# IBM/AdaMML

Measured on AMD Instinct MI355X. Metric: clips/sec (train fwd+bwd) RGB+Audio AdaMML @224^2, 5 seg, higher is better.
Workload: dtype bf16

## Files before the change

adamml_amd/csrc/conv_gemm.hip:

```cpp
#include "common.h"
#include "../../include/adamml_hip.h"
#include <type_traits>
#include <stdlib.h>
#include <stdio.h>


namespace {

constexpr int BP = 128;
constexpr int BK = 32;
constexpr int NTHREADS = 256;

struct ConvP {
    const bf16_t* x;
    const bf16_t* w;
    const float* in_scale;
    const float* in_shift;
    bf16_t* y;
    double* stats;
    int N, H, W, Cin, OH, OW, Cout, KH, KW, stride, pad, up, up_shift, act, accumulate;
    int P, K, cin_shift, n_ptiles, n_ctiles, tpb;
    size_t gx, gy;
    int in_gstride;
    const bf16_t* bn_z;
    const float* bn_vec;
    int bn_act;
    const bf16_t* res_out;
    const uint8_t* res_mask;
    int res_act;
    const bf16_t* bn_z2;
    const float* bn_vec2;
    double* stats2;
    const bf16_t* x2;
    const float* aff;
    bf16_t* side;
    const bf16_t* xb;
    int K1, C2;
    size_t gw;
    const float* epi_add;
    const float* id_scale;
    const float* id_shift;
    int id_gstride;
    uint8_t* mask_out;
    const bf16_t* pf_a;
    const float* pf_scale;
    const float* pf_shift;
    float* pf_ws;
    int pf_act, pf_gs, pf_nsplit;
    int wK;
    int cls_nt;
    unsigned cls_code;
    int oH, oW, o_ph, o_pw;
    int tp_nblk, tp_Q;
    bf16_t* tp_y;
    uint16_t* tp_code;
};

__device__ __forceinline__ int lds_off(int row, int chunk) {
    return row * 64 + ((chunk ^ (((row >> 3) & 1) << 1)) << 4);
}

template <int N, class F>
__device__ __forceinline__ void static_for(F&& f) {
    if constexpr (N > 0) {
        static_for<N - 1>(f);
        f(std::integral_constant<int, N - 1>{});
    }
}

template <int CH>
__device__ __forceinline__ int tr_swz(int row) {
    if (CH >= 128) return ((row & 3) | (((row >> 3) & 1) << 2)) << 2;
    return (((row >> 1) & 1) | (((row >> 3) & 1) << 1)) << 2;
}

__device__ const uint4 g_zero_page[4] = {};

__device__ __forceinline__ void glds16(const void* gsrc, unsigned lds_dst_uniform) {
    unsigned keep;
    asm volatile("s_mov_b32 %0, m0\n\ts_mov_b32 m0, %2\n\ts_nop 0\n\tglobal_load_lds_dwordx4 %1, off\n\ts_mov_b32 m0, %0"
                 : "=&s"(keep) : "v"(gsrc), "s"(lds_dst_uniform) : "memory");
}

constexpr int conv_gemm_wg_per_cu(int BC, int MODE, int PD, bool RES, bool DUAL, bool CAT, bool FADD, bool GLDS, int EID, int EPI) {
    if (RES || DUAL || CAT || EID) return 2;
    const int n = PD == 1 ? (BC == 128 ? 3 : 4) : (BC == 128 ? 2 : 3);
    const bool fewer = (MODE == 2 && !(BC == 128 && PD == 3)) || FADD ||
                       (BC == 64 && PD == 1 && ((EPI == 1 && !(MODE == 0 && GLDS)) || (EPI == 2 && MODE == 1))) ||
                       (BC == 128 && MODE == 1 && EPI == 2 && !GLDS);
    return fewer ? n - 1 : n;
}

template <int BC, int MODE, int PD, bool RES = false, bool DUAL = false, bool CAT = false, bool FADD = false, bool GLDS = false, int EID = 0,
          bool LZF = false, int EPI = -1, bool PF = false, int TP = 0>
__global__ __launch_bounds__(NTHREADS, conv_gemm_wg_per_cu(BC, MODE, PD, RES, DUAL, CAT, FADD, GLDS, EID, EPI)) void conv_gemm_kernel(ConvP p) {
    static_assert(TP == 0 || (FADD && EID && MODE == 0 && BC == 128 && (TP == 2 || TP == 4 || TP == 8)), "TP: FADD + EID, 128-wide cout tiles");
    constexpr int PPF = TP ? BP / TP : BP;
    constexpr int WCT = BC / 32;
    constexpr int WROWS = BC / 64;
    constexpr int TILE_BYTES = (BP + BC) * 64;
    constexpr int EPI_BYTES = BP * (BC * 2 + 16);
    constexpr int NBUF = GLDS ? 3 : 2;
    constexpr int STAGE_BYTES = (NBUF * TILE_BYTES) > EPI_BYTES ? (NBUF * TILE_BYTES) : EPI_BYTES;
    constexpr int NSR = (FADD || EPI == 0) ? 1 : 4;
    constexpr int CS_BYTES = NSR * 2 * BC * 4;
    constexpr int CS2_OFF = STAGE_BYTES + CS_BYTES + (MODE == 0 ? 0 : 256) + (MODE == 3 ? BP * 4 + 16 : 0);
    constexpr int VEC_MAXK = 1024;
    constexpr int VEC_OFF = CS2_OFF + (RES ? CS_BYTES : 0);
    constexpr int LZF_MAXK = 512;
    constexpr int PF_C = 64;
    constexpr int PF_OFF = (VEC_OFF + (LZF ? 2 * LZF_MAXK * 4 : (MODE == 0 && !GLDS) ? (DUAL ? 3 : 2) * VEC_MAXK * 4 : 0) + 1023) / 1024 * 1024;
    constexpr int SMEM_BYTES = PF ? PF_OFF + BP * PF_C * 2 : VEC_OFF + (LZF ? 2 * LZF_MAXK * 4 : (MODE == 0 && !GLDS) ? (DUAL ? 3 : 2) * VEC_MAXK * 4 : 0);
    __shared__ __attribute__((aligned(1024))) char smem[SMEM_BYTES];

    {
        const int g = blockIdx.y;
        p.x += (size_t)g * p.gx;
        p.y += (size_t)g * p.gy;
        if (p.stats) p.stats += (size_t)g * ADAMML_STAT_SLOTS * 2 * p.Cout;
        if (p.in_scale) { p.in_scale += (size_t)g * p.in_gstride; p.in_shift += (size_t)g * p.in_gstride; }
        if (p.bn_z) { p.bn_z += (size_t)g * p.gy; p.bn_vec += (size_t)g * 4 * p.Cout; }
        if (CAT) {
            p.xb += (size_t)g * (p.gx / p.K1) * p.C2;
            p.w += (size_t)g * p.gw;
            p.epi_add += (size_t)g * p.Cout;
        }
        if (DUAL) {
            p.x2 += (size_t)g * p.gx;
            p.aff += (size_t)g * 3 * p.K;
            if (p.side) p.side += (size_t)g * p.gx;
        }
        if (FADD) {
            p.bn_vec += (size_t)g * 4 * p.Cout;
            if (p.res_out) p.res_out += (size_t)g * p.gy;
            if (p.mask_out) p.mask_out += ((size_t)g * p.gy) >> 3;
            if (p.id_scale) { p.id_scale += (size_t)g * p.id_gstride; p.id_shift += (size_t)g * p.id_gstride; }
            if (TP) { p.tp_y += (size_t)g * (p.gy >> 1); if (p.tp_code) p.tp_code += ((size_t)g * (p.gy >> 1)) >> 3; }
        }
        if (PF) {
            p.pf_a += (size_t)g * p.P * PF_C;
            if (p.pf_scale) { p.pf_scale += (size_t)g * p.pf_gs; p.pf_shift += (size_t)g * p.pf_gs; }
        }
        if (RES) {
            p.res_out += (size_t)g * p.gy;
            if (p.res_mask) p.res_mask += ((size_t)g * p.gy) >> 3;
            if (p.bn_z2) { p.bn_z2 += (size_t)g * p.gy; p.bn_vec2 += (size_t)g * 4 * p.Cout; p.stats2 += (size_t)g * ADAMML_STAT_SLOTS * 2 * p.Cout; }
        }
    }
    const int tid = threadIdx.x;
    float* s_vec = reinterpret_cast<float*>(smem + (MODE == 0 ? VEC_OFF : 0));
    const int nvec = CAT ? p.C2 : p.K;
    const bool vec_lds = MODE == 0 && nvec <= VEC_MAXK && (DUAL || p.in_scale != nullptr);
    if (LZF) {
        const int kpad = (p.K + BK - 1) / BK * BK;
        for (int i = tid; i < kpad; i += NTHREADS) {
            s_vec[i] = i < p.K ? p.in_scale[i] : 0.f;
            s_vec[LZF_MAXK + i] = i < p.K ? p.in_shift[i] : 0.f;
        }
        __syncthreads();
    } else
    if (vec_lds) {
        if (DUAL) {
            for (int i = tid; i < 3 * p.K; i += NTHREADS) s_vec[i] = p.aff[i];
        } else {
            for (int i = tid; i < nvec; i += NTHREADS) { s_vec[i] = p.in_scale[i]; s_vec[nvec + i] = p.in_shift[i]; }
        }
        __syncthreads();
    }
    const int lane = tid & 63;
    const int wave = tid >> 6;
    const int wp = wave & 1;
    const int wc = wave >> 1;

    const int nwg = gridDim.x;
    int bid = blockIdx.x;
    {
        const int q = nwg >> 3, r = nwg & 7, xcd = bid & 7, idx = bid >> 3;
        bid = (xcd < r ? xcd * (q + 1) : r * (q + 1) + (xcd - r) * q) + idx;
    }
    const int ctile = bid % p.n_ctiles;
    const int pgrp = bid / p.n_ctiles;
    const int c0 = ctile * BC;

    const int chunk = tid & 3;
    const int row_a = tid >> 2;
    int* s_tapoff = reinterpret_cast<int*>(smem + STAGE_BYTES + CS_BYTES);
    int* s_wtap = s_tapoff + 64;
    int* s_orow = s_wtap + 4;
    if (MODE == 1) {
        if (tid < p.KH * p.KW) {
            const int kh = tid / p.KW, kw = tid - kh * p.KW;
            s_tapoff[tid] = (kh * p.W + kw) * p.Cin;
        }
    }
    if (MODE == 3) {
        if (tid < p.cls_nt) {
            const unsigned code = (p.cls_code >> (8 * tid)) & 0xffu;
            s_tapoff[tid] = ((int)(code & 1) * p.W + (int)((code >> 1) & 1)) * p.Cin;
            s_wtap[tid] = (int)(code >> 2) * p.Cin;
        }
    }
    const bf16_t* wrow[WROWS];
    bool w_ok[WROWS];
#pragma unroll
    for (int r = 0; r < WROWS; ++r) {
        int co = c0 + row_a + r * 64;
        w_ok[r] = co < p.Cout;
        wrow[r] = p.w + (size_t)(w_ok[r] ? co : 0) * p.wK;
    }
    const int li = lane & 15, lg = lane >> 4;
    constexpr int CROW = BC * 2 + 16;
    static_assert(BP * CROW <= STAGE_BYTES, "epilogue tile must fit the staging buffers");
    float* cs = reinterpret_cast<float*>(smem + STAGE_BYTES);
    float* cs2 = reinterpret_cast<float*>(smem + CS2_OFF);
    const bool second = RES && p.bn_z2 != nullptr;
    const bool epi_bnz = EPI < 0 ? p.bn_z != nullptr : EPI == 1;
    const bool epi_acc = EPI < 0 ? p.accumulate != 0 : (EPI == 2 && p.accumulate != 0);
    if (p.stats) {
        for (int i = tid; i < NSR * 2 * BC; i += NTHREADS) cs[i] = 0.f;
        if (second)
            for (int i = tid; i < NSR * 2 * BC; i += NTHREADS) cs2[i] = 0.f;
    }
    constexpr int CPR = BC / 8;
    constexpr int RSTEP = NTHREADS / CPR;
    const int ech = tid % CPR, erow0 = tid / CPR;
    const int eco = c0 + ech * 8;

    f32x4 pacc[PF ? 4 : 1][PF ? 2 : 1];
// ... 492 lines not shown
                if constexpr (EID != 0) {
                    dr[j] = eid[b0 + j];
                    mbits[j] = embits[b0 + j];
                } else {
                if (p.bn_z) zr[j] = __builtin_nontemporal_load(reinterpret_cast<const bf16x8*>(p.bn_z + pr[j]));
                if (p.accumulate) dr[j] = __builtin_nontemporal_load(reinterpret_cast<const bf16x8*>(p.y + pr[j]));
                if (p.res_mask) mbits[j] = p.res_mask[pr[j] >> 3];
                else orr[j] = __builtin_nontemporal_load(reinterpret_cast<const bf16x8*>(p.res_out + pr[j]));
                if (second) z2r[j] = __builtin_nontemporal_load(reinterpret_cast<const bf16x8*>(p.bn_z2 + pr[j]));
                }
            }
#pragma unroll
            for (int j = 0; j < EB; ++j) {
                const int r = erow0 + (b0 + j) * RSTEP;
                f32x8 f = bf8_to_f32(*reinterpret_cast<const bf16x8*>(smem + r * CROW + ech * 16));
                if (EID || p.accumulate) f += bf8_to_f32(dr[j]);
                if (EID || p.res_mask) {
#pragma unroll
                    for (int i = 0; i < 8; ++i) f[i] = (mbits[j] >> i) & 1u ? f[i] : 0.f;
                } else {
                    const f32x8 ov = bf8_to_f32(orr[EID ? 0 : j]);
#pragma unroll
                    for (int i = 0; i < 8; ++i) f[i] *= mask_act(ov[i], rlo, rhi);
                }
                const bf16x8 v = f32_to_bf8(f);
                if (ok[j]) *reinterpret_cast<bf16x8*>(p.y + pr[j]) = v;
                if constexpr (PF)
                    *reinterpret_cast<bf16x8*>(smem + r * CROW + ech * 16) = ok[j] ? v : bf16x8{0, 0, 0, 0, 0, 0, 0, 0};
                const float keep = ok[j] ? 1.f : 0.f;
                f = bf8_to_f32(v) * keep;
                esum += f;
                if constexpr (EID == 0) {
                if (p.bn_z) {
                    const f32x8 zv = bf8_to_f32(zr[j]);
#pragma unroll
                    for (int i = 0; i < 8; ++i) esq[i] += f[i] * (zv[i] - mu[i]) * is[i];
                }
                if (second) {
                    const f32x8 z2 = bf8_to_f32(z2r[j]);
#pragma unroll
                    for (int i = 0; i < 8; ++i) esq2[i] += f[i] * (z2[i] - mu2[i]) * is2[i];
                }
                }
            }
        }
        }
    } else if (eco < p.Cout && epi_bnz) {
        const f32x8 sc = load_f32x8(p.bn_vec + eco), sh = load_f32x8(p.bn_vec + p.Cout + eco);
        const f32x8 mu = load_f32x8(p.bn_vec + 2 * p.Cout + eco), is = load_f32x8(p.bn_vec + 3 * p.Cout + eco);
        f32x8 cadd;
#pragma unroll
        for (int i = 0; i < 8; ++i) cadd[i] = 0.f;
        if (CAT) cadd = load_f32x8(p.epi_add + eco);
        constexpr int NRZ = BP / RSTEP, EBZ = (EPI == 1 || CAT || DUAL) ? (NRZ < 4 ? NRZ : 4) : 1;
#pragma unroll 1
        for (int b0 = 0; b0 < NRZ; b0 += EBZ) {
            bf16x8 zrow[EBZ];
#pragma unroll
            for (int j = 0; j < EBZ; ++j) {
                const int r = erow0 + (b0 + j) * RSTEP;
                const int rc = p0 + r < p.P ? r : 0;
                const size_t pp = MODE == 3 ? (size_t)s_orow[rc] : (size_t)(p0 + rc);
                zrow[j] = *reinterpret_cast<const bf16x8*>(p.bn_z + pp * p.Cout + eco);
            }
#pragma unroll
            for (int j = 0; j < EBZ; ++j) {
                const int r = erow0 + (b0 + j) * RSTEP;
                if (p0 + r < p.P) {
                    const size_t pp = MODE == 3 ? (size_t)s_orow[r] : (size_t)(p0 + r);
                    f32x8 f = bf8_to_f32(*reinterpret_cast<const bf16x8*>(smem + r * CROW + ech * 16)) + cadd;
                    const f32x8 zv = bf8_to_f32(zrow[j]);
#pragma unroll
                    for (int i = 0; i < 8; ++i) f[i] *= act_mask(fmaf(zv[i], sc[i], sh[i]), p.bn_act);
                    const bf16x8 v = f32_to_bf8(f);
                    *reinterpret_cast<bf16x8*>(p.y + pp * p.Cout + eco) = v;
                    f = bf8_to_f32(v);
                    esum += f;
#pragma unroll
                    for (int i = 0; i < 8; ++i) esq[i] += f[i] * (zv[i] - mu[i]) * is[i];
                }
            }
        }
    } else if (eco < p.Cout) {
        constexpr int NRA = BP / RSTEP, EBA = (EPI == 2 || CAT || DUAL) ? (NRA < 4 ? NRA : 4) : 1;
#pragma unroll 1
        for (int b0 = 0; b0 < NRA; b0 += EBA) {
            bf16x8 arow[EBA];
            if (epi_acc) {
#pragma unroll
                for (int j = 0; j < EBA; ++j) {
                    const int r = erow0 + (b0 + j) * RSTEP;
                    const int rc = p0 + r < p.P ? r : 0;
                    const size_t pp = MODE == 3 ? (size_t)s_orow[rc] : (size_t)(p0 + rc);
                    arow[j] = *reinterpret_cast<const bf16x8*>(p.y + pp * p.Cout + eco);
                }
            }
#pragma unroll
            for (int j = 0; j < EBA; ++j) {
                const int r = erow0 + (b0 + j) * RSTEP;
                if (p0 + r < p.P) {
                    const size_t pp = MODE == 3 ? (size_t)s_orow[r] : (size_t)(p0 + r);
                    bf16x8 v = *reinterpret_cast<const bf16x8*>(smem + r * CROW + ech * 16);
                    f32x8 f = bf8_to_f32(v);
                    if (CAT) {
                        f += load_f32x8(p.epi_add + eco);
                        v = f32_to_bf8(f);
                    }
// ... 67 lines not shown
            }
        };
        static_assert(NSR == 4 || EPI == 0 || FADD, "VALU-folded sums need one row per wave");
        fold(esum, esq, cs);
        if (second) fold(esum, esq2, cs2);
    }
    if constexpr (PF) {
        __syncthreads();
        const int trow = 8 * lg + (li >> 2), tq = li & 3;
        const int x_lo = tr_swz<64>(trow), x_hi = tr_swz<64>(trow + 4);
        const float plo = p.pf_scale ? act_lo(p.pf_act) : -INFINITY, phi = p.pf_scale ? act_hi(p.pf_act) : INFINITY;
#pragma unroll
        for (int ks = 0; ks < BP / 32; ++ks) {
            bf16x8 fa[4], fb[2];
#pragma unroll
            for (int t = 0; t < 4; ++t) {
                const char* fp = smem + (ks * 32 + trow) * CROW + (wp * 64 + t * 16 + 4 * tq) * 2;
                union { s16x4 h[2]; bf16x8 v; } f;
                f.h[0] = __builtin_amdgcn_ds_read_tr16_b64_v4i16((__attribute__((address_space(3))) s16x4*)(fp));
                f.h[1] = __builtin_amdgcn_ds_read_tr16_b64_v4i16((__attribute__((address_space(3))) s16x4*)(fp + 4 * CROW));
                fa[t] = f.v;
            }
#pragma unroll
            for (int t = 0; t < 2; ++t) {
                const char* base = smem + PF_OFF + ks * 32 * 128;
                const int u = (wc * 32 + t * 16) / 4 + tq;
                union { s16x4 h[2]; bf16x8 v; } f;
                f.h[0] = __builtin_amdgcn_ds_read_tr16_b64_v4i16((__attribute__((address_space(3))) s16x4*)(base + trow * 128 + ((u ^ x_lo) << 3)));
                f.h[1] = __builtin_amdgcn_ds_read_tr16_b64_v4i16((__attribute__((address_space(3))) s16x4*)(base + (trow + 4) * 128 + ((u ^ x_hi) << 3)));
                f32x8 q = bf8_to_f32(f.v);
#pragma unroll
                for (int i = 0; i < 8; ++i) q[i] = clamp_act(fmaf(q[i], pfs[t], pfh[t]), plo, phi);
                fb[t] = f32_to_bf8(q);
            }
#pragma unroll
            for (int mt = 0; mt < 4; ++mt)
#pragma unroll
                for (int nt = 0; nt < 2; ++nt) pacc[mt][nt] = __builtin_amdgcn_mfma_f32_16x16x32_bf16(fa[mt], fb[nt], pacc[mt][nt], 0, 0, 0);
        }
    }
    __syncthreads();
    }
    if constexpr (PF) {
        float* out = p.pf_ws + (((size_t)blockIdx.y * p.n_ctiles + ctile) * p.pf_nsplit + pgrp) * (BC * PF_C);
#pragma unroll
        for (int mt = 0; mt < 4; ++mt)
#pragma unroll
            for (int nt = 0; nt < 2; ++nt)
#pragma unroll
                for (int r = 0; r < 4; ++r) out[(size_t)(wp * 64 + mt * 16 + lg * 4 + r) * PF_C + wc * 32 + nt * 16 + li] = pacc[mt][nt][r];
    }
    if (p.stats) {
        __syncthreads();
        const unsigned slot = blockIdx.x & (ADAMML_STAT_SLOTS - 1);
        for (int i = tid; i < 2 * BC; i += NTHREADS) {
            const int c = i < BC ? i : i - BC;
            if (c0 + c < p.Cout) {
                const size_t e = (i < BC ? 0 : (size_t)p.Cout) + c0 + c;
                float v = cs[i];
#pragma unroll
                for (int w = 1; w < NSR; ++w) v += cs[w * 2 * BC + i];
                stat_publish(p.stats + e, 2 * (size_t)p.Cout, slot, v);
                if (second) {
                    float v2 = cs2[i];
#pragma unroll
                    for (int w = 1; w < NSR; ++w) v2 += cs2[w * 2 * BC + i];
                    stat_publish(p.stats2 + e, 2 * (size_t)p.Cout, slot, v2);
                }
            }
        }
    }
}

struct WgradP {
    const bf16_t* dz;
    const bf16_t* x;
    const float* in_scale;
    const float* in_shift;
    float* dw;
    float* ws;
    size_t dw_numel;
    int nsplit;
    int N, H, W, Cin, OH, OW, Cout, KH, KW, stride, pad, act, cin_true;
    int P, pix_per_block, n_cotiles, n_tiles, cin_shift, NK;
    size_t gdz, gx;
    int in_gstride;
    const float* dz_scale;
    const float* dz_shift;
    int dz_act, dz_gstride;
};


template <int BM, int BN, int WPD = 1, bool LZ = false>
__global__ __launch_bounds__(NTHREADS) void conv_wgrad_kernel(WgradP p) {
    constexpr int AROW = BM * 2;
    constexpr int BROW = BN * 2;
    constexpr int TILE_BYTES = 32 * (AROW + BROW);
    constexpr int MT = BM / 32, NT = BN / 32;
    __shared__ __attribute__((aligned(16))) char smem[2 * TILE_BYTES];

    const int lb = (int)xcd_contiguous(blockIdx.x, gridDim.x);
    const int tile = lb % p.n_tiles;
    const int unit = lb / p.n_tiles;
    const int split = unit % p.nsplit, grp = unit / p.nsplit;
    p.dz += (size_t)grp * p.gdz;
    p.x += (size_t)grp * p.gx;
    if (p.in_scale) { p.in_scale += (size_t)grp * p.in_gstride; p.in_shift += (size_t)grp * p.in_gstride; }
// ... 553 lines not shown
    }
}

void launch_wgrad_reduce(const float* ws, float* dw, size_t n, int nsplit, int taps, int cin, int store, int groups, hipStream_t stream) {
    static const bool wide = !(getenv("ADAMML_REDUCE4") && getenv("ADAMML_REDUCE4")[0] == '0');
    if (wide && n % 4 == 0 && (reinterpret_cast<uintptr_t>(ws) & 15) == 0)
        hipLaunchKernelGGL(wgrad_reduce4_kernel, dim3((unsigned)((n / 4 + 15) / 16), groups), dim3(256), 0, stream, ws, dw, n, nsplit, taps, cin, store);
    else
        hipLaunchKernelGGL(wgrad_reduce_kernel, dim3((unsigned)((n + 15) / 16), groups), dim3(256), 0, stream, ws, dw, n, nsplit, taps, cin, store);
}

int ilog2_exact(int v) {
    int s = 0;
    while ((1 << s) < v) ++s;
    return (1 << s) == v ? s : -1;
}

}

bool adamml_conv3x3_c64_supported(const adamml_conv_desc_t* d);
bool adamml_conv1x1_narrow_fwd_supported(const adamml_conv_desc_t* d);
bool adamml_conv1x1_narrow_wgrad_supported(const adamml_conv_desc_t* d, int cin_true);
bool adamml_conv1x1_narrow_dual_supported(const adamml_conv_desc_t* d);
bool adamml_conv1x1_narrow_dgrad_epi_supported(const adamml_conv_desc_t* d);
int adamml_conv1x1_narrow_dgrad_epi_launch(const adamml_conv_desc_t* d, const void* dz, const void* w_packed, void* dx, const void* z_in,
                                           const float* bn_vec, int act, double* sums, hipStream_t stream);
int adamml_conv1x1_narrow_dual_launch(const adamml_conv_desc_t* d, const void* g, const void* z, const float* aff, void* dz_side,
                                      const void* w_dgrad_packed, void* dx, int accumulate, const void* z_in, const float* bn_vec, int act,
                                      double* sums, hipStream_t stream);
int adamml_conv1x1_narrow_wgrad_launch(const adamml_conv_desc_t* d, const void* dz, const void* x, const float* in_scale, const float* in_shift,
                                       float* ws, int max_blocks_per_group, int* nblk_out, hipStream_t stream);
int adamml_conv1x1_narrow_fwd_launch(const adamml_conv_desc_t* d, const void* x, const void* w_packed, const float* in_scale, const float* in_shift,
                                     void* y, double* stats, hipStream_t stream);
int adamml_conv3x3_c64_launch(const adamml_conv_desc_t* d, const void* x, const void* w_packed, const float* in_scale,
                              const float* in_shift, void* y, double* stats, const void* bn_z, const float* bn_vec, int bn_act,
                              hipStream_t stream);
bool adamml_conv1x1_wide_expand_supported(const adamml_conv_desc_t* d);
int adamml_conv1x1_wide_expand_launch(const adamml_conv_desc_t* d, const void* x, const void* w_packed, const float* in_scale, const float* in_shift,
                                      void* y, double* stats, hipStream_t stream);

bool adamml_conv3x3_c64_wgrad_supported(const adamml_conv_desc_t* d, int cin_true);
int adamml_conv3x3_c64_wgrad_blocks(const adamml_conv_desc_t* d, int* tpb_out);
int adamml_conv3x3_c64_wgrad_launch(const adamml_conv_desc_t* d, const void* dz, const void* x, const float* in_scale,
                                    const float* in_shift, float* ws, hipStream_t stream);

struct DgradClass { int nt; unsigned code; int ph, pw, OHc, OWc; };
struct ResEpi { const void* res_out; const uint8_t* res_mask; int res_act; const void* bn_z2; const float* bn_vec2; double* stats2; };
struct DualIn { const void* z; const float* aff; void* side; };
struct CatIn { const void* xb; int C2; size_t gw; const float* epi_add; };
struct PfIn { const void* a; const float* scale; const float* shift; int act, gs, C; float* out; void* ws; size_t ws_bytes; };
struct FaddEpi { const float* vec; const void* idn; const float* id_scale; const float* id_shift; int id_gstride; int act; uint8_t* mask_out;
                 int tp_frames; void* tp_y; uint16_t* tp_code; };

static int conv_launch(const adamml_conv_desc_t* d, const void* x, const void* w_packed, const float* in_scale,
                       const float* in_shift, void* y, double* stats, const void* bn_z, const float* bn_vec, int bn_act,
                       hipStream_t stream, const DgradClass* cls = nullptr, const ResEpi* res = nullptr, const DualIn* dual = nullptr,
                       const CatIn* cat = nullptr, const FaddEpi* fadd = nullptr, const PfIn* pf = nullptr) {
    if (!d || !x || !w_packed || !y) return adamml_set_error(ADAMML_EINVAL, "conv_fwd: null argument");
    if (d->Cin % 8 || d->Cout % 8) return adamml_set_error(ADAMML_EINVAL, "conv_fwd: channels must be multiples of 8 (Cin=%d Cout=%d)", d->Cin, d->Cout);
    if (!cls && !fadd && adamml_conv3x3_c64_supported(d))
        return adamml_conv3x3_c64_launch(d, x, w_packed, in_scale, in_shift, y, stats, bn_z, bn_vec, bn_act, stream);
    if (!cls && !fadd && !res && !dual && !cat && !pf && !bn_z && adamml_conv1x1_narrow_fwd_supported(d))
        return adamml_conv1x1_narrow_fwd_launch(d, x, w_packed, in_scale, in_shift, y, stats, stream);
    if (!cls && !fadd && !res && !dual && !cat && !pf && !bn_z && !(d->accumulate && in_scale) && adamml_conv1x1_wide_expand_supported(d))
        return adamml_conv1x1_wide_expand_launch(d, x, w_packed, in_scale, in_shift, y, stats, stream);
    if (!cls && !fadd && !res && !dual && !cat && !pf && !in_scale && (bn_z ? stats != nullptr && !d->accumulate : d->accumulate != 0) &&
        adamml_conv1x1_narrow_dgrad_epi_supported(d))
        return adamml_conv1x1_narrow_dgrad_epi_launch(d, x, w_packed, y, bn_z, bn_vec, bn_act, stats, stream);
    ConvP p;
    p.x = (const bf16_t*)x; p.w = (const bf16_t*)w_packed; p.in_scale = in_scale; p.in_shift = in_shift;
    p.y = (bf16_t*)y; p.stats = stats;
    p.bn_z = (const bf16_t*)bn_z; p.bn_vec = bn_vec; p.bn_act = bn_act;
    p.res_out = res ? (const bf16_t*)res->res_out : nullptr; p.res_act = res ? res->res_act : 0;
    p.res_mask = res ? res->res_mask : nullptr;
    p.bn_z2 = res ? (const bf16_t*)res->bn_z2 : nullptr; p.bn_vec2 = res ? res->bn_vec2 : nullptr; p.stats2 = res ? res->stats2 : nullptr;
    p.x2 = dual ? (const bf16_t*)dual->z : nullptr; p.aff = dual ? dual->aff : nullptr; p.side = dual ? (bf16_t*)dual->side : nullptr;
    p.xb = cat ? (const bf16_t*)cat->xb : nullptr; p.K1 = d->Cin; p.C2 = cat ? cat->C2 : 0; p.gw = cat ? cat->gw : 0;
    p.epi_add = cat ? cat->epi_add : nullptr;
    p.id_scale = fadd ? fadd->id_scale : nullptr; p.id_shift = fadd ? fadd->id_shift : nullptr; p.id_gstride = fadd ? fadd->id_gstride : 0;
    p.mask_out = fadd ? fadd->mask_out : nullptr;
    p.tp_nblk = p.tp_Q = 0; p.tp_y = nullptr; p.tp_code = nullptr;
    p.pf_a = nullptr; p.pf_scale = p.pf_shift = nullptr; p.pf_ws = nullptr; p.pf_act = p.pf_gs = p.pf_nsplit = 0;
    if (fadd) { p.bn_vec = fadd->vec; p.res_out = (const bf16_t*)fadd->idn; p.res_act = fadd->act; }
    const int groups = d->groups < 1 ? 1 : d->groups;
    p.gx = (size_t)d->N * d->H * d->W * d->Cin;
    p.gy = (size_t)d->N * d->OH * d->OW * d->Cout;
    p.in_gstride = d->in_gstride;
    p.N = d->N; p.H = d->H; p.W = d->W; p.Cin = d->Cin; p.OH = d->OH; p.OW = d->OW; p.Cout = d->Cout;
    p.KH = d->KH; p.KW = d->KW; p.stride = d->stride; p.pad = d->pad; p.up = d->up < 1 ? 1 : d->up;
    p.up_shift = ilog2_exact(p.up);
    if (p.up_shift < 0) return adamml_set_error(ADAMML_EUNSUPPORTED, "conv_fwd: up=%d is not a power of two", p.up);
    p.act = d->act; p.accumulate = d->accumulate;
    p.P = d->N * d->OH * d->OW; p.K = d->KH * d->KW * d->Cin;
    if (cat) {
        if (d->KH * d->KW != 1 || d->stride != 1 || (d->up > 1) || d->Cin % BK || cat->C2 % 8 || cls || res || dual)
            return adamml_set_error(ADAMML_EUNSUPPORTED, "conv_bwd_data_alg: 1x1 / stride-1 convs with Cout %% 32 == 0 only");
        p.K = d->Cin + cat->C2;
    }
    p.wK = p.K;
    p.cls_nt = 0; p.cls_code = 0; p.oH = d->OH; p.oW = d->OW; p.o_ph = p.o_pw = 0;
    if (cls) {
        p.cls_nt = cls->nt; p.cls_code = cls->code; p.o_ph = cls->ph; p.o_pw = cls->pw;
        p.OH = cls->OHc; p.OW = cls->OWc;
        p.P = d->N * cls->OHc * cls->OWc;
        p.K = cls->nt * d->Cin;
    }
    const bool multitap = d->KH * d->KW > 1 || cls;
    p.cin_shift = 0;
    if (multitap) {
        p.cin_shift = ilog2_exact(d->Cin);
        if (p.cin_shift < 0) return adamml_set_error(ADAMML_EUNSUPPORTED, "conv_fwd: KxK conv needs power-of-two Cin (got %d)", d->Cin);
    }
    if (p.P <= 0) return ADAMML_OK;
    bool narrow = d->Cout <= 64 || (d->Cout % 128 != 0 && d->Cout < 256);
    if (!narrow && (long)ceil_div(p.P, BP) * ceil_div(d->Cout, 128) * groups < 512) narrow = true;
    const int tp = fadd ? fadd->tp_frames : 0;
    if (tp) narrow = false;
    const int BC = narrow ? 64 : 128;
    p.n_ptiles = ceil_div(p.P, BP);
    if (tp) {
        p.tp_Q = d->OH * d->OW;
        p.tp_nblk = ceil_div(p.tp_Q, BP / tp);
        p.n_ptiles = (d->N / tp) * p.tp_nblk;
        p.tp_y = (bf16_t*)fadd->tp_y; p.tp_code = fadd->tp_code;
    }
    p.n_ctiles = ceil_div(d->Cout, BC);
    p.tpb = (int)((long)p.n_ptiles * p.n_ctiles * groups / 2048);
    if (p.tpb < 1) p.tpb = 1;
    if (p.tpb > 8) p.tpb = 8;
    if (pf) {
        const long target = 1536;
        long nsp = target / ((long)p.n_ctiles * groups);
        if (nsp < 1) nsp = 1;
        p.tpb = (int)ceil_div(p.n_ptiles, (int)nsp);
        if (p.tpb < 1) p.tpb = 1;
    }
    dim3 grid(ceil_div(p.n_ptiles, p.tpb) * p.n_ctiles, groups), block(NTHREADS);
    const int taps = d->KH * d->KW;
    if ((long)d->N * d->H * d->W * d->Cin >= (1L << 31)) return adamml_set_error(ADAMML_EUNSUPPORTED, "conv_fwd: input tensor exceeds 2^31 elements");
    const int mode = cls ? 3 : (p.up > 1 ? 2 : (multitap ? (taps <= 64 ? 1 : 2) : 0));
    if (mode == 2 && !multitap) { p.cin_shift = 30; }
    const int nk = ceil_div(p.K, BK);
    const bool deep = (long)grid.x * grid.y <= 768 && nk >= 8 && mode != 1;
    if (fadd) {
        if (mode != 0 || res || dual || cat || stats) return adamml_set_error(ADAMML_EUNSUPPORTED, "conv_fwd_bn_add: only 1x1 / stride-1 convs");
        static const int fadd_glds = getenv("ADAMML_FADD_GLDS") ? atoi(getenv("ADAMML_FADD_GLDS")) : 2;
        if (fadd_glds && (!in_scale || p.K <= 512)) {
            const bool eid = fadd_glds > 1 && p.res_out;
            if (tp) {
#define LAUNCH_TP(TV)                                                                                                                                        \
                do {                                                                                                                                         \
                    if (in_scale) hipLaunchKernelGGL((conv_gemm_kernel<128, 0, 1, false, false, false, true, true, 1, true, -1, false, TV>), grid, block, 0, stream, p);  \
                    else hipLaunchKernelGGL((conv_gemm_kernel<128, 0, 1, false, false, false, true, true, 1, false, -1, false, TV>), grid, block, 0, stream, p);         \
                } while (0)
                if (tp == 8) LAUNCH_TP(8); else if (tp == 4) LAUNCH_TP(4); else LAUNCH_TP(2);
#undef LAUNCH_TP
                return adamml_check_launch("conv_fwd_bn_add_tpool");
            }
#define LAUNCH_FADD(BCV)                                                                                                                   \
            do {                                                                                                                           \
                if (in_scale) {                                                                                                            \
                    if (eid) hipLaunchKernelGGL((conv_gemm_kernel<BCV, 0, 1, false, false, false, true, true, 1, true>), grid, block, 0, stream, p);  \
                    else hipLaunchKernelGGL((conv_gemm_kernel<BCV, 0, 1, false, false, false, true, true, 0, true>), grid, block, 0, stream, p);      \
                } else {                                                                                                                   \
                    if (eid) hipLaunchKernelGGL((conv_gemm_kernel<BCV, 0, 1, false, false, false, true, true, 1, false>), grid, block, 0, stream, p); \
                    else hipLaunchKernelGGL((conv_gemm_kernel<BCV, 0, 1, false, false, false, true, true, 0, false>), grid, block, 0, stream, p);     \
                }                                                                                                                          \
            } while (0)
            if (BC == 64) LAUNCH_FADD(64); else LAUNCH_FADD(128);
#undef LAUNCH_FADD
        } else
        if (tp) return adamml_set_error(ADAMML_EUNSUPPORTED, "conv_fwd_bn_add_tpool: needs the LDS-DMA kernel (K <= 512 for a lazy input)");
        else
        if (BC == 64) hipLaunchKernelGGL((conv_gemm_kernel<64, 0, 1, false, false, false, true>), grid, block, 0, stream, p);
        else hipLaunchKernelGGL((conv_gemm_kernel<128, 0, 1, false, false, false, true>), grid, block, 0, stream, p);
        return adamml_check_launch("conv_fwd_bn_add");
    }
    if (res) {
        if (mode != 0) return adamml_set_error(ADAMML_EUNSUPPORTED, "conv_bwd_data_res: only 1x1 / stride-1 convs");
        static const bool res_eid = !(getenv("ADAMML_RES_EID") && getenv("ADAMML_RES_EID")[0] == '0');
        if (pf) {
            if (BC != 128 || d->Cout % 128 || pf->C != 64 || in_scale || !p.res_mask || !p.accumulate || p.bn_z || p.bn_z2 || !stats)
                return adamml_set_error(ADAMML_EUNSUPPORTED, "conv_bwd_data_res_prod: needs Cout %% 128 == 0, a 64-channel product operand, "
                                                             "the accumulate + 1-bit-mask + sum(g')-only form");
            p.pf_nsplit = ceil_div(p.n_ptiles, p.tpb);
            const size_t need = (size_t)groups * p.n_ctiles * p.pf_nsplit * 128 * 64 * sizeof(float);
            if (!pf->ws || pf->ws_bytes < need) return adamml_set_error(ADAMML_EINVAL, "conv_bwd_data_res_prod: workspace too small (need %zu bytes)", need);
            p.pf_a = (const bf16_t*)pf->a; p.pf_scale = pf->scale; p.pf_shift = pf->scale ? pf->shift : nullptr; p.pf_act = pf->act; p.pf_gs = pf->gs;
            p.pf_ws = (float*)pf->ws;
            hipLaunchKernelGGL((conv_gemm_kernel<128, 0, 1, true, false, false, false, true, 1, false, -1, true>), grid, block, 0, stream, p);
// ... 154 lines not shown
}

extern "C" int adamml_conv_fwd_bn_add_tpool(const adamml_conv_desc_t* d, const void* x, const void* w_packed, const float* in_scale,
                                            const float* in_shift, const float* bn_vec, const void* idn, const float* id_scale,
                                            const float* id_shift, int id_gstride, int act, int frames, void* pooled, uint16_t* code,
                                            hipStream_t stream) {
    if (!adamml_conv_fwd_bn_add_tpool_supported(d, frames, act, in_scale != nullptr))
        return adamml_set_error(ADAMML_EUNSUPPORTED, "conv_fwd_bn_add_tpool: 1x1 / stride-1 conv, Cout %% 128 == 0, ReLU, 2 / 4 / 8 frames per clip");
    if (!bn_vec || !idn || !pooled) return adamml_set_error(ADAMML_EINVAL, "conv_fwd_bn_add_tpool: null argument");
    if (adamml_conv1x1_fadd_tpool_stream_supported(d, frames))
        return adamml_conv1x1_fadd_tpool_stream_launch(d, x, w_packed, in_scale, in_shift, bn_vec, idn, id_scale, id_shift, id_gstride, act, frames, pooled,
                                                       code, stream);
    if (adamml_conv1x1_fadd_tpool_supported(d, frames))
        return adamml_conv1x1_fadd_tpool_launch(d, x, w_packed, in_scale, in_shift, bn_vec, idn, id_scale, id_shift, id_gstride, act, frames, pooled, code,
                                                stream);
    FaddEpi f{bn_vec, idn, id_scale, id_shift, id_gstride, act, nullptr, frames, pooled, code};
    return conv_launch(d, x, w_packed, in_scale, in_shift, pooled, nullptr, nullptr, nullptr, 0, stream, nullptr, nullptr, nullptr, nullptr, &f);
}

__global__ void gram_stats_kernel(const bf16_t* w, const float* G, const float* s, double* sums, int Cout, int Cin) {
    const int co = blockIdx.x, g = blockIdx.y, lane = threadIdx.x;
    const bf16_t* wr = w + (size_t)co * Cin;
    const float* Gg = G + (size_t)g * Cin * Cin;
    const float* sg = s + (size_t)g * Cin;
    double a1 = 0.0, a2 = 0.0;
    for (int ci = lane; ci < Cin; ci += 64) {
        const double wi = (double)__builtin_bit_cast(float, (unsigned)wr[ci] << 16);
        const float* col = Gg + ci;
        double t0 = 0.0, t1 = 0.0, t2 = 0.0, t3 = 0.0;
        for (int cj = 0; cj < Cin; cj += 4) {
            t0 += (double)col[(size_t)cj * Cin] * (double)__builtin_bit_cast(float, (unsigned)wr[cj] << 16);
            t1 += (double)col[(size_t)(cj + 1) * Cin] * (double)__builtin_bit_cast(float, (unsigned)wr[cj + 1] << 16);
            t2 += (double)col[(size_t)(cj + 2) * Cin] * (double)__builtin_bit_cast(float, (unsigned)wr[cj + 2] << 16);
            t3 += (double)col[(size_t)(cj + 3) * Cin] * (double)__builtin_bit_cast(float, (unsigned)wr[cj + 3] << 16);
        }
        a1 += wi * (double)sg[ci];
        a2 += wi * ((t0 + t1) + (t2 + t3));
    }
#pragma unroll
    for (int off = 32; off >= 1; off >>= 1) { a1 += __shfl_xor(a1, off, 64); a2 += __shfl_xor(a2, off, 64); }
    if (lane == 0) {
        sums[(size_t)g * 2 * Cout + co] = a1;
        sums[(size_t)g * 2 * Cout + Cout + co] = a2;
    }
}

extern "C" int adamml_gram_stats(const void* w_packed, const float* G, const float* s, double* sums, int Cout, int Cin, int groups,
                                 hipStream_t stream) {
    if (!w_packed || !G || !s || !sums || Cout < 1 || Cin < 4 || (Cin & 3) || groups < 1) return adamml_set_error(ADAMML_EINVAL, "gram_stats: bad arguments (Cin must be a multiple of 4)");
    hipLaunchKernelGGL(gram_stats_kernel, dim3(Cout, groups), dim3(64), 0, stream, (const bf16_t*)w_packed, G, s, sums, Cout, Cin);
    return adamml_check_launch("gram_stats");
}

static int conv_dgrad_stride2(const adamml_conv_desc_t* d, const void* dz, const void* w, void* dx, int accumulate, double* sums,
                              const void* z_in, const float* bn_vec, int act, hipStream_t stream) {
    adamml_conv_desc_t g = *d;
    g.N = d->N; g.H = d->OH; g.W = d->OW; g.Cin = d->Cout;
    g.OH = d->H; g.OW = d->W; g.Cout = d->Cin;
    g.stride = 1; g.up = 1; g.pad = 0;
    g.act = ACT_NONE; g.accumulate = accumulate; g.in_gstride = 0;
    const int taps = d->KH * d->KW;
    for (int ph = 0; ph < 2; ++ph)
        for (int pw = 0; pw < 2; ++pw) {
            DgradClass c;
            c.nt = 0; c.code = 0; c.ph = ph; c.pw = pw;
            c.OHc = (d->H - ph + 1) / 2; c.OWc = (d->W - pw + 1) / 2;
            if (c.OHc <= 0 || c.OWc <= 0) continue;
            for (int kh = 0; kh < d->KH; ++kh) {
                if ((ph + d->pad - kh) & 1) continue;
                const int dh = (ph + d->pad - kh) / 2;
                for (int kw = 0; kw < d->KW; ++kw) {
                    if ((pw + d->pad - kw) & 1) continue;
                    const int dw = (pw + d->pad - kw) / 2;
                    const unsigned wt = (unsigned)(taps - 1 - (kh * d->KW + kw));
                    c.code |= ((unsigned)dh | ((unsigned)dw << 1) | (wt << 2)) << (8 * c.nt);
                    ++c.nt;
                }
            }
            if (c.nt == 0 && accumulate) continue;
            int rc = conv_launch(&g, dz, w, nullptr, nullptr, dx, sums, z_in, bn_vec, act, stream, &c);
            if (rc) return rc;
        }
    return ADAMML_OK;
}

static bool dgrad_stride2_ok(const adamml_conv_desc_t* d) {
    const bool k3 = d->KH == 3 && d->KW == 3 && d->pad == 1, k1 = d->KH == 1 && d->KW == 1 && d->pad == 0;
    return d->stride == 2 && (k3 || k1) && (d->up <= 1) && ilog2_exact(d->Cout) >= 0 &&
           d->OH == (d->H + 2 * d->pad - d->KH) / 2 + 1 && d->OW == (d->W + 2 * d->pad - d->KW) / 2 + 1;
}

extern "C" int adamml_conv_bwd_data_bn(const adamml_conv_desc_t* d, const void* dz, const void* w_dgrad_packed, void* dx,
                                       const void* z_in, const float* bn_vec, int act, double* sums, hipStream_t stream) {
    if (!d || !z_in || !bn_vec || !sums) return adamml_set_error(ADAMML_EINVAL, "conv_bwd_data_bn: null argument");
    if (dgrad_stride2_ok(d)) return conv_dgrad_stride2(d, dz, w_dgrad_packed, dx, 0, sums, z_in, bn_vec, act, stream);
    adamml_conv_desc_t g = *d;
    g.N = d->N; g.H = d->OH; g.W = d->OW; g.Cin = d->Cout;
    g.OH = d->H; g.OW = d->W; g.Cout = d->Cin;
    g.stride = 1; g.up = d->stride; g.pad = d->KH - 1 - d->pad;
    g.act = ACT_NONE; g.accumulate = 0; g.in_gstride = 0;
    return conv_launch(&g, dz, w_dgrad_packed, nullptr, nullptr, dx, sums, z_in, bn_vec, act, stream);
}

extern "C" int adamml_conv_bwd_data_dual_supported(const adamml_conv_desc_t* d) {
    return d && d->KH == 1 && d->KW == 1 && d->stride == 1 && d->pad == 0 && d->Cout <= 512 && d->Cin % 8 == 0 && d->Cout % 8 == 0 ? 1 : 0;
}

extern "C" int adamml_conv_bwd_data_dual(const adamml_conv_desc_t* d, const void* g, const void* z, const float* aff, void* dz_side,
                                         const void* w_dgrad_packed, void* dx, int accumulate, const void* z_in, const float* bn_vec,
                                         int act, double* sums, hipStream_t stream) {
    if (!d || !g || !z || !aff) return adamml_set_error(ADAMML_EINVAL, "conv_bwd_data_dual: null argument");
    if (!adamml_conv_bwd_data_dual_supported(d))
        return adamml_set_error(ADAMML_EUNSUPPORTED, "conv_bwd_data_dual: only 1x1 / stride-1 convs with Cout <= 512");
    if ((z_in != nullptr) != (bn_vec != nullptr) || (z_in != nullptr) != (sums != nullptr))
        return adamml_set_error(ADAMML_EINVAL, "conv_bwd_data_dual: incomplete BatchNorm epilogue operands");
    if (z_in && accumulate) return adamml_set_error(ADAMML_EUNSUPPORTED, "conv_bwd_data_dual: the BatchNorm epilogue does not accumulate");
    if (adamml_conv1x1_narrow_dual_supported(d))
        return adamml_conv1x1_narrow_dual_launch(d, g, z, aff, dz_side, w_dgrad_packed, dx, accumulate, z_in, bn_vec, act, sums, stream);
    adamml_conv_desc_t gd = *d;
    gd.N = d->N; gd.H = d->OH; gd.W = d->OW; gd.Cin = d->Cout;
    gd.OH = d->H; gd.OW = d->W; gd.Cout = d->Cin;
    gd.stride = 1; gd.up = 1; gd.pad = 0;
    gd.act = ACT_NONE; gd.accumulate = accumulate ? 1 : 0; gd.in_gstride = 0;
    DualIn di{z, aff, dz_side};
    return conv_launch(&gd, g, w_dgrad_packed, nullptr, nullptr, dx, sums, z_in, bn_vec, act, stream, nullptr, nullptr, &di);
}

bool adamml_alg_stream_supported(int Cout, int Cin);
int adamml_alg_stream_launch(const adamml_conv_desc_t* d, const void* g, const void* a, const float* a_scale, const float* a_shift,
                             const void* w_alg, const float* epi_add, void* dx, int accumulate, const void* z_in, const float* bn_vec,
                             int act, double* sums, hipStream_t stream);
static bool alg_stream_enabled() {
    static int on = -1;
    if (on < 0) { const char* e = getenv("ADAMML_ALG_STREAM"); on = (e && e[0] == '0') ? 0 : 1; }
    return on == 1;
}

__global__ void alg_pack_kernel(const float* w, const float* aff, const float* m_pre, bf16_t* wp, float* cadd, int Cout, int Cin, int groups) {
    const int K = Cout + Cin;
    const size_t total = (size_t)groups * Cin * K;
    for (size_t e = (size_t)blockIdx.x * blockDim.x + threadIdx.x; e < total; e += (size_t)gridDim.x * blockDim.x) {
        const int k = (int)(e % K);
// ... 386 lines not shown
```

include/adamml_hip.h:

```cpp
#ifndef ADAMML_HIP_H
#define ADAMML_HIP_H
#include <stddef.h>
#include <stdint.h>
#ifdef __cplusplus
extern "C" {
#endif

typedef struct ihipStream_t* hipStream_t;
typedef struct ihipEvent_t* hipEvent_t;

#define ADAMML_API __attribute__((visibility("default")))

#define ADAMML_STAT_SLOTS 32

#define ADAMML_ACT_NONE 0
#define ADAMML_ACT_RELU 1
#define ADAMML_ACT_RELU6 2

typedef struct {
    int32_t N, H, W, Cin;
    int32_t OH, OW, Cout;
    int32_t KH, KW, stride, pad;
    int32_t up;
    int32_t act;
    int32_t accumulate;
    int32_t groups;
    int32_t in_gstride;
} adamml_conv_desc_t;

ADAMML_API int adamml_version(void);
ADAMML_API const char* adamml_last_error_string(void);
ADAMML_API int adamml_set_deterministic(int on);
ADAMML_API int adamml_get_deterministic(void);

ADAMML_API int adamml_conv_fwd(const adamml_conv_desc_t* d, const void* x, const void* w_packed, const float* in_scale,
                    const float* in_shift, void* y, double* stats, hipStream_t stream);
ADAMML_API int adamml_conv_fused_input_supported(const adamml_conv_desc_t* d);
ADAMML_API int adamml_conv1x1_narrow_supported(const adamml_conv_desc_t* d, int kind);
ADAMML_API int adamml_conv1x1_wide_supported(const adamml_conv_desc_t* d, int kind);
ADAMML_API int adamml_conv_fwd_bn_add_supported(const adamml_conv_desc_t* d);
ADAMML_API int adamml_conv_fwd_bn_add_streams(const adamml_conv_desc_t* d);
ADAMML_API int adamml_conv_fwd_bn_add(const adamml_conv_desc_t* d, const void* x, const void* w_packed, const float* in_scale, const float* in_shift,
                           const float* bn_vec, const void* idn, const float* id_scale, const float* id_shift, int id_gstride, int act,
                           void* out, uint8_t* mask_out, hipStream_t stream);
ADAMML_API int adamml_conv_fwd_bn_add_next_supported(const adamml_conv_desc_t* d, int next_cout);
ADAMML_API int adamml_conv_fwd_bn_add_next(const adamml_conv_desc_t* d, const void* x, const void* w_packed, const float* in_scale, const float* in_shift,
                                const float* bn_vec, const void* idn, const float* id_scale, const float* id_shift, int id_gstride, int act,
                                void* out, uint8_t* mask_out, const void* w_next, void* y_next, double* stats_next, hipStream_t stream);
ADAMML_API int adamml_conv_fwd_bn_add_tpool_supported(const adamml_conv_desc_t* d, int frames, int act, int lazy_input);
ADAMML_API int adamml_conv_fwd_bn_add_tpool_streams(const adamml_conv_desc_t* d, int frames);
ADAMML_API int adamml_conv_fwd_bn_add_tpool(const adamml_conv_desc_t* d, const void* x, const void* w_packed, const float* in_scale, const float* in_shift,
                                 const float* bn_vec, const void* idn, const float* id_scale, const float* id_shift, int id_gstride, int act,
                                 int frames, void* pooled, uint16_t* code, hipStream_t stream);
ADAMML_API int adamml_gram_stats(const void* w_packed, const float* G, const float* s, double* sums, int Cout, int Cin, int groups, hipStream_t stream);
ADAMML_API int adamml_gram_colsum_supported(int C);
ADAMML_API size_t adamml_gram_colsum_workspace(size_t P, int C, int groups);
ADAMML_API int adamml_gram_colsum(const void* x, const float* scale, const float* shift, int gstride, int act, float* G, float* s, size_t P, int C,
                       int groups, void* workspace, size_t workspace_bytes, hipStream_t stream);
ADAMML_API int adamml_conv_bwd_data(const adamml_conv_desc_t* d, const void* dz, const void* w_dgrad_packed, void* dx,
                         int accumulate, hipStream_t stream);
ADAMML_API int adamml_conv_bwd_data_bn(const adamml_conv_desc_t* d, const void* dz, const void* w_dgrad_packed, void* dx, const void* z_in,
                            const float* bn_vec, int act, double* sums, hipStream_t stream);

ADAMML_API int adamml_conv_bwd_data_dual_supported(const adamml_conv_desc_t* d);
ADAMML_API int adamml_bn_bwd_affine(const float* coef, const float* vec, float* aff, int C, int groups, hipStream_t stream);
ADAMML_API int adamml_conv_bwd_data_dual(const adamml_conv_desc_t* d, const void* g, const void* z, const float* aff, void* dz_side,
                              const void* w_dgrad_packed, void* dx, int accumulate, const void* z_in, const float* bn_vec, int act,
                              double* sums, hipStream_t stream);

ADAMML_API int adamml_conv_bwd_weight_grouped(const adamml_conv_desc_t* d, const void* dz, const float* dz_scale, const float* dz_shift, int dz_act,
                                   int dz_gstride, const void* x, const float* in_scale, const float* in_shift, float* out, int cin_true,
                                   void* workspace, size_t workspace_bytes, hipStream_t stream);
ADAMML_API int adamml_lazy_colsum(const void* x, const float* scale, const float* shift, int gstride, int act, float* s, size_t P, int C, int groups,
                       hipStream_t stream);
ADAMML_API int adamml_alg_sumfix(const float* w, const float* P, const float* vec, double* sums, int Cout, int Cin, int groups, hipStream_t stream);
ADAMML_API int adamml_alg_pack(const float* w, const float* aff, const float* m_pre, void* w_alg, float* epi_add, int Cout, int Cin, int groups,
                    hipStream_t stream);
ADAMML_API int adamml_alg_wgrad_combine(const float* w, const float* aff, const float* P, const float* G, const float* wg_pre, const float* s, float* dw,
                             int Cout, int Cin, int groups, hipStream_t stream);
ADAMML_API int adamml_conv_bwd_data_alg(const adamml_conv_desc_t* d, const void* g, const void* a, const float* a_scale, const float* a_shift,
                             const void* w_alg, const float* epi_add, void* dx, int accumulate, const void* z_in, const float* bn_vec,
                             int act, double* sums, hipStream_t stream);

ADAMML_API int adamml_conv_bwd_data_res_supported(const adamml_conv_desc_t* d);
ADAMML_API int adamml_conv_bwd_data_res_streams(const adamml_conv_desc_t* d);
ADAMML_API int adamml_conv_bwd_data_res(const adamml_conv_desc_t* d, const void* dz, const void* w_dgrad_packed, void* dx,
                             int accumulate, const void* res_out, const uint8_t* res_mask, int res_act, const void* z_a, const float* vec_a,
                             double* sums_a, const void* z_b, const float* vec_b, double* sums_b, hipStream_t stream);

ADAMML_API int adamml_conv_bwd_data_res_prod_supported(const adamml_conv_desc_t* d, int a_channels);
ADAMML_API size_t adamml_conv_bwd_data_res_prod_workspace(const adamml_conv_desc_t* d);
ADAMML_API int adamml_conv_bwd_data_res_prod_streams(const adamml_conv_desc_t* d, int a_channels);
ADAMML_API int adamml_conv_bwd_data_res_prod(const adamml_conv_desc_t* d, const void* dz, const void* w_dgrad_packed, void* dx, const uint8_t* res_mask,
                                  int res_act, double* sums_a, const void* a, const float* a_scale, const float* a_shift, int a_act,
                                  int a_gstride, int a_channels, float* prod, void* workspace, size_t workspace_bytes, hipStream_t stream);

ADAMML_API size_t adamml_conv_bwd_weight_workspace(const adamml_conv_desc_t* d, int cin_true);
ADAMML_API int adamml_conv_bwd_weight(const adamml_conv_desc_t* d, const void* dz, const void* x, const float* in_scale,
                           const float* in_shift, float* dw, int cin_true, void* workspace, size_t workspace_bytes,
                           hipStream_t stream);
ADAMML_API int adamml_pack_conv_weight(const float* w, void* out, int cout, int cin_true, int cin_pad, int kh, int kw, int mode,
                            hipStream_t stream);

ADAMML_API int adamml_conv_stem_supported(const adamml_conv_desc_t* d);
ADAMML_API int adamml_pack_stem_weight(const float* w, void* out, int cout, int cin_true, hipStream_t stream);
ADAMML_API int adamml_conv_stem_fwd(const adamml_conv_desc_t* d, const void* x, const void* w_stem_packed, void* y, double* stats,
                         hipStream_t stream);
ADAMML_API size_t adamml_conv_stem_bwd_weight_workspace(const adamml_conv_desc_t* d);
ADAMML_API int adamml_conv_stem_bwd_weight(const adamml_conv_desc_t* d, const void* dz, const void* x, float* dw, int cin_true,
                                void* workspace, size_t workspace_bytes, hipStream_t stream);

// ... 141 lines not shown
```

Before: 3464.

## Merge stride-2 dgrad parity-class launches into one grid with per-class block ranges

Stride-2 3x3 backward-data previously launched one conv kernel per output parity class, up to four launches. Now a single launch covers all classes: each class gets a block range in the grid, sorted by tap count so heavier classes start first, and each block reads its class parameters from a small table in the kernel arguments. This removes per-launch overhead and the tail idling between small launches. It also widens the BN-epilogue z-row prefetch batch for this mode, which raises register pressure. A padding of each class range to multiples of 8 adds a few idle blocks, and the feature can be turned off with an environment variable.

```diff
diff --git a/adamml_amd/csrc/conv_gemm.hip b/adamml_amd/csrc/conv_gemm.hip
--- a/adamml_amd/csrc/conv_gemm.hip
+++ b/adamml_amd/csrc/conv_gemm.hip
@@ -1,6 +1,7 @@
 #include "common.h"
 #include "../../include/adamml_hip.h"
 #include <type_traits>
+#include <algorithm>
 #include <stdlib.h>
 #include <stdio.h>
 
@@ -51,6 +52,8 @@
     int cls_nt;
     unsigned cls_code;
     int oH, oW, o_ph, o_pw;
+    int ncls;
+    struct Cls { unsigned code; int nt, ph, pw, OH, OW, P, K, n_ptiles, tpb, b0, nwg; } cls[4];
     int tp_nblk, tp_Q;
     bf16_t* tp_y;
     uint16_t* tp_code;
@@ -113,6 +116,30 @@
     constexpr int SMEM_BYTES = PF ? PF_OFF + BP * PF_C * 2 : VEC_OFF + (LZF ? 2 * LZF_MAXK * 4 : (MODE == 0 && !GLDS) ? (DUAL ? 3 : 2) * VEC_MAXK * 4 : 0);
     __shared__ __attribute__((aligned(1024))) char smem[SMEM_BYTES];
 
+    int blk = blockIdx.x, nwg = gridDim.x;
+    if constexpr (MODE == 3) {
+        if (p.ncls > 0) {
+            int c = 0;
+#pragma unroll
+            for (int i = 1; i < 4; ++i)
+                if (i < p.ncls && blk >= p.cls[i].b0) c = i;
+            unsigned code = p.cls[0].code;
+            int nt = p.cls[0].nt, ph = p.cls[0].ph, pw = p.cls[0].pw, oh = p.cls[0].OH, ow = p.cls[0].OW, np = p.cls[0].P, kk = p.cls[0].K;
+            int npt = p.cls[0].n_ptiles, tpb = p.cls[0].tpb, b0 = p.cls[0].b0, cn = p.cls[0].nwg;
+#pragma unroll
+            for (int i = 1; i < 4; ++i)
+                if (c == i) {
+                    code = p.cls[i].code; nt = p.cls[i].nt; ph = p.cls[i].ph; pw = p.cls[i].pw; oh = p.cls[i].OH; ow = p.cls[i].OW;
+                    np = p.cls[i].P; kk = p.cls[i].K; npt = p.cls[i].n_ptiles; tpb = p.cls[i].tpb; b0 = p.cls[i].b0; cn = p.cls[i].nwg;
+                }
+            blk -= b0;
+            nwg = cn;
+            if (blk >= nwg) return;
+            p.cls_code = code; p.cls_nt = nt; p.o_ph = ph; p.o_pw = pw; p.OH = oh; p.OW = ow; p.P = np; p.K = kk;
+            p.n_ptiles = npt; p.tpb = tpb;
+        }
+    }
+
     {
         const int g = blockIdx.y;
         p.x += (size_t)g * p.gx;
@@ -172,8 +199,7 @@
     const int wp = wave & 1;
     const int wc = wave >> 1;
 
-    const int nwg = gridDim.x;
-    int bid = blockIdx.x;
+    int bid = blk;
     {
         const int q = nwg >> 3, r = nwg & 7, xcd = bid & 7, idx = bid >> 3;
         bid = (xcd < r ? xcd * (q + 1) : r * (q + 1) + (xcd - r) * q) + idx;
@@ -772,7 +798,8 @@
 #pragma unroll
         for (int i = 0; i < 8; ++i) cadd[i] = 0.f;
         if (CAT) cadd = load_f32x8(p.epi_add + eco);
-        constexpr int NRZ = BP / RSTEP, EBZ = (EPI == 1 || CAT || DUAL) ? (NRZ < 4 ? NRZ : 4) : 1;
+        constexpr int EBZ_MAX = (EPI == 1 && GLDS && MODE == 3) ? 8 : 4;
+        constexpr int NRZ = BP / RSTEP, EBZ = (EPI == 1 || CAT || DUAL) ? (NRZ < EBZ_MAX ? NRZ : EBZ_MAX) : 1;
 #pragma unroll 1
         for (int b0 = 0; b0 < NRZ; b0 += EBZ) {
             bf16x8 zrow[EBZ];
@@ -946,7 +973,7 @@
     }
     if (p.stats) {
         __syncthreads();
-        const unsigned slot = blockIdx.x & (ADAMML_STAT_SLOTS - 1);
+        const unsigned slot = blk & (ADAMML_STAT_SLOTS - 1);
         for (int i = tid; i < 2 * BC; i += NTHREADS) {
             const int c = i < BC ? i : i - BC;
             if (c0 + c < p.Cout) {
@@ -1606,10 +1633,14 @@
 struct FaddEpi { const float* vec; const void* idn; const float* id_scale; const float* id_shift; int id_gstride; int act; uint8_t* mask_out;
                  int tp_frames; void* tp_y; uint16_t* tp_code; };
 
+static bool conv_narrow_tile(int Cout, int P, int groups) {
+    return Cout <= 64 || (Cout % 128 != 0 && Cout < 256) || (long)ceil_div(P, BP) * ceil_div(Cout, 128) * groups < 512;
+}
+
 static int conv_launch(const adamml_conv_desc_t* d, const void* x, const void* w_packed, const float* in_scale,
                        const float* in_shift, void* y, double* stats, const void* bn_z, const float* bn_vec, int bn_act,
                        hipStream_t stream, const DgradClass* cls = nullptr, const ResEpi* res = nullptr, const DualIn* dual = nullptr,
-                       const CatIn* cat = nullptr, const FaddEpi* fadd = nullptr, const PfIn* pf = nullptr) {
+                       const CatIn* cat = nullptr, const FaddEpi* fadd = nullptr, const PfIn* pf = nullptr, int ncls = 1) {
     if (!d || !x || !w_packed || !y) return adamml_set_error(ADAMML_EINVAL, "conv_fwd: null argument");
     if (d->Cin % 8 || d->Cout % 8) return adamml_set_error(ADAMML_EINVAL, "conv_fwd: channels must be multiples of 8 (Cin=%d Cout=%d)", d->Cin, d->Cout);
     if (!cls && !fadd && adamml_conv3x3_c64_supported(d))
@@ -1653,6 +1684,9 @@
     }
     p.wK = p.K;
     p.cls_nt = 0; p.cls_code = 0; p.oH = d->OH; p.oW = d->OW; p.o_ph = p.o_pw = 0;
+    p.ncls = 0;
+    for (ConvP::Cls& k : p.cls) k = ConvP::Cls{};
+    if (ncls < 1 || ncls > 4 || (ncls > 1 && !cls)) return adamml_set_error(ADAMML_EINVAL, "conv_bwd_data: bad parity class count %d", ncls);
     if (cls) {
         p.cls_nt = cls->nt; p.cls_code = cls->code; p.o_ph = cls->ph; p.o_pw = cls->pw;
         p.OH = cls->OHc; p.OW = cls->OWc;
@@ -1666,8 +1700,7 @@
         if (p.cin_shift < 0) return adamml_set_error(ADAMML_EUNSUPPORTED, "conv_fwd: KxK conv needs power-of-two Cin (got %d)", d->Cin);
     }
     if (p.P <= 0) return ADAMML_OK;
-    bool narrow = d->Cout <= 64 || (d->Cout % 128 != 0 && d->Cout < 256);
-    if (!narrow && (long)ceil_div(p.P, BP) * ceil_div(d->Cout, 128) * groups < 512) narrow = true;
+    bool narrow = conv_narrow_tile(d->Cout, p.P, groups);
     const int tp = fadd ? fadd->tp_frames : 0;
     if (tp) narrow = false;
     const int BC = narrow ? 64 : 128;
@@ -1690,6 +1723,25 @@
         if (p.tpb < 1) p.tpb = 1;
     }
     dim3 grid(ceil_div(p.n_ptiles, p.tpb) * p.n_ctiles, groups), block(NTHREADS);
+    if (ncls > 1) {
+        int b0 = 0;
+        for (int c = 0; c < ncls; ++c) {
+            ConvP::Cls& k = p.cls[c];
+            k.code = cls[c].code; k.nt = cls[c].nt; k.ph = cls[c].ph; k.pw = cls[c].pw; k.OH = cls[c].OHc; k.OW = cls[c].OWc;
+            k.P = d->N * cls[c].OHc * cls[c].OWc; k.K = cls[c].nt * d->Cin;
+            k.n_ptiles = ceil_div(k.P, BP);
+            if (k.P <= 0) return adamml_set_error(ADAMML_EINVAL, "conv_bwd_data: empty parity class");
+            if (conv_narrow_tile(d->Cout, k.P, groups) != narrow) return adamml_set_error(ADAMML_EUNSUPPORTED, "conv_bwd_data: parity classes of different tile widths");
+            k.tpb = (int)((long)k.n_ptiles * p.n_ctiles * groups / 2048);
+            if (k.tpb < 1) k.tpb = 1;
+            if (k.tpb > 8) k.tpb = 8;
+            k.nwg = ceil_div(k.n_ptiles, k.tpb) * p.n_ctiles;
+            k.b0 = b0;
+            b0 += ceil_div(k.nwg, 8) * 8;
+        }
+        p.ncls = ncls;
+        grid.x = b0;
+    }
     const int taps = d->KH * d->KW;
     if ((long)d->N * d->H * d->W * d->Cin >= (1L << 31)) return adamml_set_error(ADAMML_EUNSUPPORTED, "conv_fwd: input tensor exceeds 2^31 elements");
     const int mode = cls ? 3 : (p.up > 1 ? 2 : (multitap ? (taps <= 64 ? 1 : 2) : 0));
@@ -1950,14 +2002,9 @@
     return adamml_check_launch("gram_stats");
 }
 
-static int conv_dgrad_stride2(const adamml_conv_desc_t* d, const void* dz, const void* w, void* dx, int accumulate, double* sums,
-                              const void* z_in, const float* bn_vec, int act, hipStream_t stream) {
-    adamml_conv_desc_t g = *d;
-    g.N = d->N; g.H = d->OH; g.W = d->OW; g.Cin = d->Cout;
-    g.OH = d->H; g.OW = d->W; g.Cout = d->Cin;
-    g.stride = 1; g.up = 1; g.pad = 0;
-    g.act = ACT_NONE; g.accumulate = accumulate; g.in_gstride = 0;
+static int dgrad_stride2_classes(const adamml_conv_desc_t* d, int accumulate, DgradClass* out) {
     const int taps = d->KH * d->KW;
+    int n = 0;
     for (int ph = 0; ph < 2; ++ph)
         for (int pw = 0; pw < 2; ++pw) {
             DgradClass c;
@@ -1976,9 +2023,43 @@
                 }
             }
             if (c.nt == 0 && accumulate) continue;
-            int rc = conv_launch(&g, dz, w, nullptr, nullptr, dx, sums, z_in, bn_vec, act, stream, &c);
-            if (rc) return rc;
-        }
+            out[n++] = c;
+        }
+    return n;
+}
+
+static adamml_conv_desc_t dgrad_stride2_desc(const adamml_conv_desc_t* d, int accumulate) {
+    adamml_conv_desc_t g = *d;
+    g.N = d->N; g.H = d->OH; g.W = d->OW; g.Cin = d->Cout;
+    g.OH = d->H; g.OW = d->W; g.Cout = d->Cin;
+    g.stride = 1; g.up = 1; g.pad = 0;
+    g.act = ACT_NONE; g.accumulate = accumulate; g.in_gstride = 0;
+    return g;
+}
+
+static bool merged_ok(const adamml_conv_desc_t* d, const DgradClass* c, int n) {
+    if (d->KH != 3 || d->KW != 3 || n < 2) return false;
+    const int groups = d->groups < 1 ? 1 : d->groups;
+    for (int i = 1; i < n; ++i)
+        if (conv_narrow_tile(d->Cin, d->N * c[i].OHc * c[i].OWc, groups) != conv_narrow_tile(d->Cin, d->N * c[0].OHc * c[0].OWc, groups))
+            return false;
+    return true;
+}
+
+static int conv_dgrad_stride2(const adamml_conv_desc_t* d, const void* dz, const void* w, void* dx, int accumulate, double* sums,
+                              const void* z_in, const float* bn_vec, int act, hipStream_t stream) {
+    const adamml_conv_desc_t g = dgrad_stride2_desc(d, accumulate);
+    DgradClass c[4];
+    const int n = dgrad_stride2_classes(d, accumulate, c);
+    const char* env = getenv("ADAMML_DGRAD_S2_MERGE");
+    if (!(env && env[0] == '0') && merged_ok(d, c, n)) {
+        std::stable_sort(c, c + n, [](const DgradClass& a, const DgradClass& b) { return a.nt > b.nt; });
+        return conv_launch(&g, dz, w, nullptr, nullptr, dx, sums, z_in, bn_vec, act, stream, c, nullptr, nullptr, nullptr, nullptr, nullptr, n);
+    }
+    for (int i = 0; i < n; ++i) {
+        int rc = conv_launch(&g, dz, w, nullptr, nullptr, dx, sums, z_in, bn_vec, act, stream, &c[i]);
+        if (rc) return rc;
+    }
     return ADAMML_OK;
 }
 
@@ -1986,6 +2067,13 @@
     const bool k3 = d->KH == 3 && d->KW == 3 && d->pad == 1, k1 = d->KH == 1 && d->KW == 1 && d->pad == 0;
     return d->stride == 2 && (k3 || k1) && (d->up <= 1) && ilog2_exact(d->Cout) >= 0 &&
            d->OH == (d->H + 2 * d->pad - d->KH) / 2 + 1 && d->OW == (d->W + 2 * d->pad - d->KW) / 2 + 1;
+}
+
+extern "C" int adamml_conv_dgrad_stride2_merged_supported(const adamml_conv_desc_t* d) {
+    if (!d || !dgrad_stride2_ok(d)) return 0;
+    DgradClass c[4];
+    const int n = dgrad_stride2_classes(d, 0, c);
+    return merged_ok(d, c, n) ? 1 : 0;
 }
 
 extern "C" int adamml_conv_bwd_data_bn(const adamml_conv_desc_t* d, const void* dz, const void* w_dgrad_packed, void* dx,
diff --git a/include/adamml_hip.h b/include/adamml_hip.h
--- a/include/adamml_hip.h
+++ b/include/adamml_hip.h
@@ -57,6 +57,7 @@
 ADAMML_API size_t adamml_gram_colsum_workspace(size_t P, int C, int groups);
 ADAMML_API int adamml_gram_colsum(const void* x, const float* scale, const float* shift, int gstride, int act, float* G, float* s, size_t P, int C,
                        int groups, void* workspace, size_t workspace_bytes, hipStream_t stream);
+ADAMML_API int adamml_conv_dgrad_stride2_merged_supported(const adamml_conv_desc_t* d);
 ADAMML_API int adamml_conv_bwd_data(const adamml_conv_desc_t* d, const void* dz, const void* w_dgrad_packed, void* dx,
                          int accumulate, hipStream_t stream);
 ADAMML_API int adamml_conv_bwd_data_bn(const adamml_conv_desc_t* d, const void* dz, const void* w_dgrad_packed, void* dx, const void* z_in,
```

New measurement: 3450 (median of 2 runs). Within noise of the previous version (-0.4%).
